# romanoshiliarhopoulos/Backgammon-Engine

Measured on AMD Instinct MI355X. Metric: self-play env steps/sec @65k concurrent games, higher is better.
Workload: dtype f32; 1 GPU; config3: 65 536 concurrent games per MI355X, greedy 198->128->1 value net (tdgammonNEW100k weights), auto-reset, Philox dice; games_per_gpu=65536, burnin_steps=160, parallelism=shard1, games_finished=2250605

## Files before the change

backgammon-engine_amd/csrc/bg_eval.h:

```cpp
#pragma once
#include "bg_board.h"
#include "bg_td_plan.h"
#include "bg_step_plan.h"

namespace bg {

constexpr int N_IN = 198, N_HID = 128;
constexpr int N_PARAMS = N_HID * N_IN + N_HID + N_HID + 1;
constexpr int K_STEPS = N_IN / 2;
constexpr int EVAL_LDS_BYTES = K_STEPS * 64 * 16;

typedef float floatx16 __attribute__((ext_vector_type(16)));

__device__ __forceinline__ float fast_sigmoid(float x)
{
    return __builtin_amdgcn_rcpf(1.0f + __builtin_amdgcn_exp2f(-1.44269504088896340736f * x));
}

__device__ __forceinline__ void best_atomic_max(unsigned long long *__restrict__ best, uint32_t game, float v, uint32_t key_turn,
                                                bool valid, int width)
{
    const int lane = threadIdx.x & 63;
    uint32_t bits = __float_as_uint(v);
    bits = (key_turn >> 31) ? ~bits : bits;
// ... 14 lines not shown
    uint32_t od[2][4];
    float tail[3];
};

__device__ __forceinline__ void decode_setup(const uint32_t (&p)[8], int h, RowDecode &r)
{
#pragma unroll
    for (int q = 0; q < 2; ++q) {
        const uint32_t b0 = p[4 * q] & PTS, b1 = p[4 * q + 1] & PTS, b2 = p[4 * q + 2] & PTS, b3 = p[4 * q + 3] & PTS;
        const uint32_t ge1 = b0 | b1 | b2 | b3;
        const uint32_t ge2 = b1 | b2 | b3;
        const uint32_t ge3 = (b0 & b1) | b2 | b3;
        const uint32_t ge4 = b2 | b3;
        const uint32_t s0 = ~b0, c0 = b0;
        const uint32_t s1 = b1 ^ c0, c1 = b1 & c0;
        const uint32_t s2 = ~(b2 ^ c1), c2 = b2 | c1;
        const uint32_t s3 = ~(b3 ^ c2);
        r.ev[q] = h ? ge2 : ge1;
        r.od[q][0] = h ? (s0 & ge4) : 0u;
        r.od[q][1] = h ? (s1 & ge4) : ge3;
        r.od[q][2] = h ? (s2 & ge4) : 0u;
        r.od[q][3] = h ? (s3 & ge4) : 0u;
    }
    const Side a{{p[0], p[1], p[2], p[3]}}, b{{p[4], p[5], p[6], p[7]}};
    const int turn = (p[0] & TURN_BIT) ? 1 : 0;
    r.tail[0] = (h == turn) ? 1.0f : 0.0f;
    r.tail[1] = 0.5f * (float)(h ? count_at(b, 25) : count_at(a, 0));
    r.tail[2] = (float)(h ? count_at(b, 0) : count_at(a, 25)) / 15.0f;
}

__device__ __forceinline__ float decode_even(const RowDecode &r, int q, int i)
{
    return (float)((r.ev[q] >> (i + 1)) & 1u);
}
__device__ __forceinline__ float decode_odd(const RowDecode &r, int q, int i)
{
    const int sh = i + 1;
    const uint32_t code = ((r.od[q][0] >> sh) & 1u) | (((r.od[q][1] >> sh) & 1u) << 1) |
                          (((r.od[q][2] >> sh) & 1u) << 2) | (((r.od[q][3] >> sh) & 1u) << 3);
    return 0.5f * (float)code;
}

inline void relayout_w1_f32(const float *w1 , float *wl )
{
    for (int s = 0; s < K_STEPS; ++s)
        for (int l = 0; l < 64; ++l)
            for (int c = 0; c < 4; ++c)
                wl[(s * 64 + l) * 4 + c] = w1[(32 * c + (l & 31)) * N_IN + 2 * s + (l >> 5)];
}

constexpr int EVAL_RED_STRIDE = 33;
constexpr int EVAL_RED_FLOATS = 32 * EVAL_RED_STRIDE;
constexpr int EVAL_LDS_TOTAL = EVAL_LDS_BYTES + (EVAL_THREADS / 64) * EVAL_RED_FLOATS * 4;

template <bool HIDDEN>
__global__ __launch_bounds__(EVAL_THREADS) void eval_rows_f32_kernel(
    const uint4 *__restrict__ rows, const unsigned long long *__restrict__ n_rows_ptr, long long n_rows_imm,
    unsigned long long *__restrict__ rows_eval_counter, const float4 *__restrict__ wl, const float *__restrict__ b1, const float *__restrict__ w2,
    const float *__restrict__ b2p, float *__restrict__ values, const uint2 *__restrict__ info,
    unsigned long long *__restrict__ best, unsigned long long *__restrict__ ksteps_counter)
{
    extern __shared__ float4 sW[];
    float *sRed = reinterpret_cast<float *>(sW + K_STEPS * 64) + (threadIdx.x >> 6) * EVAL_RED_FLOATS;
    for (int i = threadIdx.x; i < K_STEPS * 64; i += EVAL_THREADS) sW[i] = wl[i];
    __syncthreads();

    long long n_rows = n_rows_imm;
    if (n_rows_ptr) { const long long c = (long long)*n_rows_ptr; n_rows = c < n_rows_imm ? c : n_rows_imm; }
    if (rows_eval_counter && blockIdx.x == 0 && threadIdx.x == 0) atomicAdd(rows_eval_counter, (unsigned long long)n_rows);
    const long long n_tiles = (n_rows + 31) >> 5;
    const int lane = threadIdx.x & 63;
    const int r = lane & 31, h = lane >> 5;
    const long long wave = (long long)blockIdx.x * (EVAL_THREADS / 64) + (threadIdx.x >> 6);
    const long long n_waves = (long long)gridDim.x * (EVAL_THREADS / 64);

    constexpr float NL2E = -1.44269504088896340736f;
    float b1s[4], w2v[4];
#pragma unroll
    for (int c = 0; c < 4; ++c) { b1s[c] = NL2E * b1[32 * c + r]; w2v[c] = w2[32 * c + r]; }
    const float b2 = *b2p;

    uint32_t ksteps = 0;
    uint4 nx0 = make_uint4(0, 0, 0, 0), nx1 = make_uint4(0, 0, 0, 0);
    if (wave < n_tiles && wave * 32 + r < n_rows) { nx0 = rows[2 * (wave * 32 + r)]; nx1 = rows[2 * (wave * 32 + r) + 1]; }

    for (long long tile = wave; tile < n_tiles; tile += n_waves) {
        const uint32_t p[8] = {nx0.x, nx0.y, nx0.z, nx0.w, nx1.x, nx1.y, nx1.z, nx1.w};
        {
            const long long nrow = (tile + n_waves) * 32 + r;
            nx0 = make_uint4(0, 0, 0, 0); nx1 = make_uint4(0, 0, 0, 0);
            if (nrow < n_rows) { nx0 = rows[2 * nrow]; nx1 = rows[2 * nrow + 1]; }
        }
        RowDecode rd;
        decode_setup(p, h, rd);

        uint32_t live[4];
        {
            const uint32_t b0a = p[0] & PTS, b1a = p[1] & PTS, b2a = p[2] & PTS, b3a = p[3] & PTS;
            const uint32_t b0b = p[4] & PTS, b1b = p[5] & PTS, b2b = p[6] & PTS, b3b = p[7] & PTS;
            live[0] = b0a | b1a | b2a | b3a;
            live[1] = (b0a & b1a) | b2a | b3a;
            live[2] = b0b | b1b | b2b | b3b;
            live[3] = (b0b & b1b) | b2b | b3b;
#pragma unroll
            for (int m = 1; m < 64; m <<= 1) {
#pragma unroll
                for (int q = 0; q < 4; ++q) live[q] |= __shfl_xor(live[q], m, 64);
            }
#pragma unroll
            for (int q = 0; q < 4; ++q) live[q] = __builtin_amdgcn_readfirstlane(live[q]) >> 1;
            ksteps += (uint32_t)(__popc(live[0]) + __popc(live[1]) + __popc(live[2]) + __popc(live[3]) + 3);
        }

        floatx16 acc0 = {0}, acc1 = {0}, acc2 = {0}, acc3 = {0};
#define BG_MFMA4(aval, WV)                                                          \
    {                                                                                \
        acc0 = __builtin_amdgcn_mfma_f32_32x32x2f32((aval), (WV).x, acc0, 0, 0, 0);    \
        acc1 = __builtin_amdgcn_mfma_f32_32x32x2f32((aval), (WV).y, acc1, 0, 0, 0);    \
        acc2 = __builtin_amdgcn_mfma_f32_32x32x2f32((aval), (WV).z, acc2, 0, 0, 0);    \
        acc3 = __builtin_amdgcn_mfma_f32_32x32x2f32((aval), (WV).w, acc3, 0, 0, 0);    \
    }
        __builtin_amdgcn_s_setprio(2);
        const float4 *wp = sW + lane;
        float4 wa = wp[0 * 64], wb = wp[1 * 64], wc = wp[2 * 64], wd = wp[3 * 64];
#pragma unroll 2
        for (int i = 0; i < 24; ++i) {
            const int nb = (4 * i + 4) * 64;
            const float4 na = wp[nb], nbb = wp[nb + 64], nc = wp[nb + 128], nd = wp[i < 23 ? nb + 192 : nb + 128];
            const float a0 = decode_even(rd, 0, i);
            const float a2 = decode_even(rd, 1, i);
            if ((live[0] >> i) & 1u) BG_MFMA4(a0, wa);
            if ((live[1] >> i) & 1u) { const float a1 = decode_odd(rd, 0, i); BG_MFMA4(a1, wb); }
            if ((live[2] >> i) & 1u) BG_MFMA4(a2, wc);
            if ((live[3] >> i) & 1u) { const float a3 = decode_odd(rd, 1, i); BG_MFMA4(a3, wd); }
            wa = na; wb = nbb; wc = nc; wd = nd;
        }
        BG_MFMA4(rd.tail[0], wa);
        BG_MFMA4(rd.tail[1], wb);
        BG_MFMA4(rd.tail[2], wc);
#undef BG_MFMA4

        __builtin_amdgcn_s_setprio(0);
        if (HIDDEN) {
            float bb[4];
#pragma unroll
            for (int c = 0; c < 4; ++c) bb[c] = b1[32 * c + r];
#pragma unroll
            for (int j = 0; j < 16; ++j) {
                const long long orow = tile * 32 + (j & 3) + 8 * (j >> 2) + 4 * h;
                if (orow < n_rows) {
                    float *o = values + orow * N_HID + r;
                    o[0] = NL2E * (acc0[j] + bb[0]); o[32] = NL2E * (acc1[j] + bb[1]);
                    o[64] = NL2E * (acc2[j] + bb[2]); o[96] = NL2E * (acc3[j] + bb[3]);
                }
            }
            continue;
        }
        float part[16];
#pragma unroll
        for (int j = 0; j < 16; ++j) {
            const float s0 = __builtin_amdgcn_rcpf(1.0f + __builtin_amdgcn_exp2f(__builtin_fmaf(acc0[j], NL2E, b1s[0])));
            const float s1 = __builtin_amdgcn_rcpf(1.0f + __builtin_amdgcn_exp2f(__builtin_fmaf(acc1[j], NL2E, b1s[1])));
            const float s2 = __builtin_amdgcn_rcpf(1.0f + __builtin_amdgcn_exp2f(__builtin_fmaf(acc2[j], NL2E, b1s[2])));
            const float s3 = __builtin_amdgcn_rcpf(1.0f + __builtin_amdgcn_exp2f(__builtin_fmaf(acc3[j], NL2E, b1s[3])));
            part[j] = w2v[0] * s0 + w2v[1] * s1 + w2v[2] * s2 + w2v[3] * s3;
        }
#pragma unroll
        for (int q = 0; q < 4; ++q)
#pragma unroll
            for (int j = 0; j < 4; ++j) sRed[r * EVAL_RED_STRIDE + 8 * q + 4 * h + j] = part[4 * q + j];
        __builtin_amdgcn_wave_barrier();
        float sum = 0.0f;
#pragma unroll
        for (int c = 0; c < 16; ++c) sum += sRed[(16 * h + c) * EVAL_RED_STRIDE + r];
        sum += __shfl_xor(sum, 32, 64);
        __builtin_amdgcn_wave_barrier();
        {
            const long long orow = tile * 32 + r;
            const bool vrow = h == 0 && orow < n_rows;
            const float v = fast_sigmoid(sum + b2);
            if (vrow) values[orow] = v;
            if (info) {
                const uint2 inf = vrow ? info[orow] : make_uint2(0u, 0u);
                best_atomic_max(best, inf.x, v, inf.y, vrow, 32);
            }
        }
    }
    __shared__ unsigned int s_ksteps;
    if (threadIdx.x == 0) s_ksteps = 0;
    __syncthreads();
    if (lane == 0 && ksteps) atomicAdd(&s_ksteps, ksteps);
    __syncthreads();
    if (ksteps_counter && threadIdx.x == 0 && s_ksteps) atomicAdd(ksteps_counter, (unsigned long long)s_ksteps);
}

#ifndef BG_DW_STRIDE
#define BG_DW_STRIDE 132
#endif
constexpr int DW_STRIDE = BG_DW_STRIDE;
#if defined(BG_ROW_LAYOUT) && BG_ROW_LAYOUT == 1
constexpr int DW_ROWS = 198;
__host__ __device__ constexpr int delta_row(int f) { return f < 192 ? (f >> 3) + 24 * (f & 7) : f; }
__host__ __device__ constexpr int delta_row_board(int point, int k8) { return point + 24 * k8; }
#else
constexpr int DW_ROWS = 9 * 24 + 6;
__host__ __device__ constexpr int delta_row(int f) { return f < 192 ? 9 * (f >> 3) + (f & 7) : 216 + (f - 192); }
__host__ __device__ constexpr int delta_row_board(int point, int k8) { return 9 * point + k8; }
#endif
constexpr int DELTA_W_FLOATS = DW_ROWS * DW_STRIDE;
constexpr int DELTA_MAX = 16;
#ifndef BG_CTR_STRIDE
#define BG_CTR_STRIDE 16
#endif
constexpr int DELTA_LDS_TOTAL = (DELTA_W_FLOATS + N_HID) * 4 + (DELTA_THREADS / 64) * DELTA_MAX * 64 * 2;

inline void relayout_w1_delta(const float *w1 , float *wt )
{
    const float NL2E = -1.44269504088896340736f;
    for (int i = 0; i < DELTA_W_FLOATS; ++i) wt[i] = 0.0f;
    for (int f = 0; f < N_IN; ++f)
        for (int n = 0; n < N_HID; ++n) {
            float w = NL2E * w1[n * N_IN + f];
            if (f >= 196) w = w / 15.0f;
            wt[delta_row(f) * DW_STRIDE + n] = 0.5f * w;
        }
}

typedef float f32x2_t __attribute__((ext_vector_type(2)));
typedef float f32x4_t __attribute__((ext_vector_type(4)));
#define BG_DA_FMA(ACC, W) "v_pk_fma_f32 " ACC ", %16, " W ", " ACC " op_sel_hi:[0,1,1]\n\t"
#define BG_DA_BODY(O0, O1, O2, O3, O4, O5, O6, O7)                                                          \
        "ds_read_b128 v[108:111], %17 offset:" #O0 "\n\t"                                                  \
        "ds_read_b128 v[112:115], %17 offset:" #O1 "\n\t"                                                  \
        "ds_read_b128 v[116:119], %17 offset:" #O2 "\n\t"                                                  \
        "ds_read_b128 v[120:123], %17 offset:" #O3 "\n\t"                                                  \
        "ds_read_b128 v[124:127], %17 offset:" #O4 "\n\t"                                                  \
        "s_waitcnt lgkmcnt(4)\n\t" BG_DA_FMA("%0", "v[108:109]") BG_DA_FMA("%1", "v[110:111]")              \
        "ds_read_b128 v[108:111], %17 offset:" #O5 "\n\t"                                                  \
        "s_waitcnt lgkmcnt(4)\n\t" BG_DA_FMA("%2", "v[112:113]") BG_DA_FMA("%3", "v[114:115]")              \
        "ds_read_b128 v[112:115], %17 offset:" #O6 "\n\t"                                                  \
        "s_waitcnt lgkmcnt(4)\n\t" BG_DA_FMA("%4", "v[116:117]") BG_DA_FMA("%5", "v[118:119]")              \
        "ds_read_b128 v[116:119], %17 offset:" #O7 "\n\t"                                                  \
        "s_waitcnt lgkmcnt(4)\n\t" BG_DA_FMA("%6", "v[120:121]") BG_DA_FMA("%7", "v[122:123]")              \
        "s_waitcnt lgkmcnt(3)\n\t" BG_DA_FMA("%8", "v[124:125]") BG_DA_FMA("%9", "v[126:127]")              \
        "s_waitcnt lgkmcnt(2)\n\t" BG_DA_FMA("%10", "v[108:109]") BG_DA_FMA("%11", "v[110:111]")            \
        "s_waitcnt lgkmcnt(1)\n\t" BG_DA_FMA("%12", "v[112:113]") BG_DA_FMA("%13", "v[114:115]")            \
        "s_waitcnt lgkmcnt(0)\n\t" BG_DA_FMA("%14", "v[116:117]") "v_pk_fma_f32 %15, %16, v[118:119], %15 op_sel_hi:[0,1,1]"
template <int OFF>
__device__ __forceinline__ void delta_apply_32(f32x2_t (&a)[16], f32x2_t d2, uint32_t lds_addr)
{
    static_assert(OFF == 0 || OFF == 128, "two halves of a 64-unit pass");
#define BG_DA_OPS                                                                                                  \
        : "+v"(a[0]), "+v"(a[1]), "+v"(a[2]), "+v"(a[3]), "+v"(a[4]), "+v"(a[5]), "+v"(a[6]), "+v"(a[7]), "+v"(a[8]),  \
          "+v"(a[9]), "+v"(a[10]), "+v"(a[11]), "+v"(a[12]), "+v"(a[13]), "+v"(a[14]), "+v"(a[15])                 \
        : "v"(d2), "v"(lds_addr)                                                                                   \
        : "v108", "v109", "v110", "v111", "v112", "v113", "v114", "v115", "v116", "v117", "v118", "v119", "v120", "v121", \
          "v122", "v123", "v124", "v125", "v126", "v127", "memory"
    if (OFF == 0) asm volatile(BG_DA_BODY(0, 16, 32, 48, 64, 80, 96, 112) BG_DA_OPS);
    else asm volatile(BG_DA_BODY(128, 144, 160, 176, 192, 208, 224, 240) BG_DA_OPS);
#undef BG_DA_OPS
}
#undef BG_DA_BODY
#undef BG_DA_FMA

__device__ __forceinline__ void delta_entry(uint32_t ent, uint32_t base, f32x2_t &d2, uint32_t &addr)
{
    float d;
    asm("v_cvt_f32_i32_sdwa %0, sext(%2) dst_sel:DWORD dst_unused:UNUSED_PAD src0_sel:BYTE_1\n\t"
        "v_mul_u32_u24_sdwa %1, %3, %2 dst_sel:DWORD dst_unused:UNUSED_PAD src0_sel:DWORD src1_sel:BYTE_0\n\t"
        "v_add_u32_e32 %1, %4, %1"
        : "=&v"(d), "=&v"(addr)
        : "v"(ent), "s"((uint32_t)(DW_STRIDE * 4)), "s"(base));
    d2.x = d;
}

__device__ __forceinline__ f32x2_t delta_sigmoid_pair(f32x2_t a, f32x2_t w, f32x2_t sum)
{
    f32x2_t e = {__builtin_amdgcn_exp2f(a.x), __builtin_amdgcn_exp2f(a.y)};
    e = e + (f32x2_t){1.0f, 1.0f};
    const f32x2_t r = {__builtin_amdgcn_rcpf(e.x), __builtin_amdgcn_rcpf(e.y)};
    return __builtin_elementwise_fma(w, r, sum);
}

#if BG_DELTA_THREADS == 1024
#define BG_DELTA_BOUNDS __launch_bounds__(DELTA_THREADS)
#else
#define BG_DELTA_BOUNDS __launch_bounds__(DELTA_THREADS, 4)
#endif
__global__ BG_DELTA_BOUNDS void eval_rows_delta_kernel(
    const uint4 *__restrict__ rows, const unsigned long long *__restrict__ n_rows_ptr, long long n_rows_imm,
    unsigned long long *__restrict__ rows_eval_counter, const float4 *__restrict__ wt, const float *__restrict__ w2,
    const float *__restrict__ b2p, const uint4 *__restrict__ root_rows, const float *__restrict__ root_hidden,
    float *__restrict__ values, const uint2 *__restrict__ info, unsigned long long *__restrict__ best,
    unsigned long long *__restrict__ delta_counter, unsigned long long *__restrict__ zero_words, int n_zero_words,
    unsigned long long *__restrict__ err_word, unsigned long long err_bit, const unsigned long long *__restrict__ n_rows_b_ptr, long long b_base)
{
    if (zero_words && blockIdx.x == 0 && (int)threadIdx.x < n_zero_words) zero_words[threadIdx.x] = 0ull;
#ifdef BG_EVAL_WGCLOCK
    const unsigned long long wg_t0 = wall_clock64();
#endif
    extern __shared__ float4 sW[];
    float *sW2 = reinterpret_cast<float *>(sW) + DELTA_W_FLOATS;
    uint16_t *sList = reinterpret_cast<uint16_t *>(sW2 + N_HID) + (threadIdx.x >> 6) * (DELTA_MAX * 64);
    for (int i = threadIdx.x; i < DELTA_W_FLOATS / 4; i += DELTA_THREADS) sW[i] = wt[i];
    if (threadIdx.x < N_HID) sW2[threadIdx.x] = w2[threadIdx.x];
    __shared__ unsigned int s_ticket;
    if (threadIdx.x == 0) s_ticket = 0;
    __syncthreads();

    long long n_rows = n_rows_imm, na1 = 0, na2 = 0, na3 = 0;
    if (n_rows_ptr) {
        const long long lim = n_rows_b_ptr ? b_base : n_rows_imm;
        const long long c = (long long)*n_rows_ptr;
        n_rows = c < lim ? c : lim;
    }
    if (n_rows_b_ptr) {
        const long long c1 = (long long)n_rows_b_ptr[0], c2 = (long long)n_rows_b_ptr[BG_CTR_STRIDE], c3 = (long long)n_rows_b_ptr[2 * BG_CTR_STRIDE];
        na1 = c1 < b_base ? c1 : b_base; na2 = c2 < b_base ? c2 : b_base; na3 = c3 < b_base ? c3 : b_base;
    }
    if (rows_eval_counter && blockIdx.x == 0 && threadIdx.x == 0) atomicAdd(rows_eval_counter, (unsigned long long)(n_rows + na1 + na2 + na3));
#ifndef BG_ARENA_ORDER
#define BG_ARENA_ORDER 123
#endif
    constexpr int AO0 = (BG_ARENA_ORDER / 1000) % 10, AO1 = (BG_ARENA_ORDER / 100) % 10, AO2 = (BG_ARENA_ORDER / 10) % 10, AO3 = BG_ARENA_ORDER % 10;
    static_assert(((1 << AO0) | (1 << AO1) | (1 << AO2) | (1 << AO3)) == 15, "a permutation of 0123");
    const long long cnt_of[4] = {n_rows, na1, na2, na3};
    const long long c0 = cnt_of[AO0], c1 = cnt_of[AO1], c2 = cnt_of[AO2], c3 = cnt_of[AO3];
    const long long t1 = (c0 + 63) >> 6, t2 = t1 + ((c1 + 63) >> 6), t3 = t2 + ((c2 + 63) >> 6);
    const long long n_tiles = t3 + ((c3 + 63) >> 6);
    auto tile_rows = [&](long long t, long long &end) -> long long {
        if (t < t1) { end = AO0 * b_base + c0; return AO0 * b_base + t * 64; }
        if (t < t2) { end = AO1 * b_base + c1; return AO1 * b_base + (t - t1) * 64; }
        if (t < t3) { end = AO2 * b_base + c2; return AO2 * b_base + (t - t2) * 64; }
        end = AO3 * b_base + c3;
        return AO3 * b_base + (t - t3) * 64;
    };
    const int lane = threadIdx.x & 63;
    int rl, inv;
    {
        const int hl = lane & 31;
        const int g = (hl < 4 || (hl >= 12 && hl < 16) || (hl >= 20 && hl < 28)) ? 0 : 1;
        const int k = hl < 4 ? hl : hl < 12 ? hl - 4 : hl < 16 ? hl - 8 : hl < 20 ? hl - 8 : hl < 28 ? hl - 12 : hl - 16;
        rl = (lane & 32) + 16 * g + k;
        const int R = lane, gg = (R >> 4) & 1, kk = R & 15;
        inv = (R & 32) + (gg == 0 ? (kk < 4 ? kk : kk < 8 ? 8 + kk : 12 + kk) : (kk < 8 ? 4 + kk : kk < 12 ? 8 + kk : 16 + kk));
    }
    const long long t_hi = n_tiles;
    auto grab = [&]() -> long long {
        unsigned int t = 0;
        if (lane == 0) t = atomicAdd(&s_ticket, 1u);
        return (long long)blockIdx.x + (long long)__builtin_amdgcn_readfirstlane(t) * (long long)gridDim.x;
    };
    const float b2 = *b2p;
    constexpr float NL2E = -1.44269504088896340736f;
    uint32_t n_delta = 0;
    bool list_overflow = false;

    uint4 nx0 = make_uint4(0, 0, 0, 0), nx1 = make_uint4(0, 0, 0, 0);
    uint2 nxi = make_uint2(0u, 0u);
    long long tile = grab();
    long long row_end = 0, row_cur = tile_rows(tile, row_end) + rl;
    if (tile < t_hi && row_cur < row_end) { nx0 = rows[2 * row_cur]; nx1 = rows[2 * row_cur + 1]; nxi = info[row_cur]; }
    uint4 nr0 = root_rows[2 * (long long)nxi.x], nr1 = root_rows[2 * (long long)nxi.x + 1];
    while (tile < t_hi) {
        const long long next_tile = grab();
        const long long row = row_cur;
        const bool valid = row < row_end;
        const uint2 inf = nxi;
        const uint4 r0 = nr0, r1 = nr1;
        const f32x4_t *ah = reinterpret_cast<const f32x4_t *>(root_hidden + (long long)inf.x * N_HID);
        const uint32_t p[8] = {nx0.x & ~TURN_BIT, nx0.y, nx0.z, nx0.w, nx1.x, nx1.y, nx1.z, nx1.w};
        const uint32_t mover = (nx0.x & TURN_BIT) ? 1u : 0u;
        const uint32_t q[8] = {valid ? r0.x & ~TURN_BIT : 0u, valid ? r0.y : 0u, valid ? r0.z : 0u, valid ? r0.w : 0u,
                               valid ? r1.x : 0u, valid ? r1.y : 0u, valid ? r1.z : 0u, valid ? r1.w : 0u};
        {
            const long long nrow = tile_rows(next_tile, row_end) + rl;
            row_cur = nrow;
            nx0 = make_uint4(0, 0, 0, 0); nx1 = make_uint4(0, 0, 0, 0); nxi = make_uint2(0u, 0u);
            if (next_tile < t_hi && nrow < row_end) { nx0 = rows[2 * nrow]; nx1 = rows[2 * nrow + 1]; nxi = info[nrow]; }
        }

        uint32_t cnt = 0;
        uint16_t *lst = sList + lane;
#pragma unroll
        for (int e = 0; e < DELTA_MAX; ++e) lst[e * 64] = 0;
#if defined(BG_ABL) && (BG_ABL & 1)
        if (p[0] == 0xFFFFFFFFu)
#endif
        {
#define BG_PUSH(F, TYPE, M)                                                                          \
    {                                                                                                \
        if (cnt < DELTA_MAX) lst[cnt * 64] = (uint16_t)((uint32_t)(F) | ((uint32_t)(((TYPE) == 1 ? 1 : 2) * (M)) & 255u) << 8); \
        ++cnt;                                                                                       \
    }
#if !defined(BG_DECODE_MOVER_FIRST) || BG_DECODE_MOVER_FIRST
#pragma unroll
        for (int pass = 0; pass < 2; ++pass) {
            const uint32_t sd = mover ^ (uint32_t)pass;
            const uint32_t b0 = sd ? p[4] : p[0], b1 = sd ? p[5] : p[1], b2 = sd ? p[6] : p[2], b3 = sd ? p[7] : p[3];
            const uint32_t c0 = sd ? q[4] : q[0], c1 = sd ? q[5] : q[1], c2 = sd ? q[6] : q[2], c3 = sd ? q[7] : q[3];
            const uint32_t diff = (b0 ^ c0) | (b1 ^ c1) | (b2 ^ c2) | (b3 ^ c3);
            if (pass == 1 && __ballot(diff != 0u) == 0ull) break;
            const uint32_t ge_new[3] = {b0 | b1 | b2 | b3, b1 | b2 | b3, (b0 & b1) | b2 | b3};
            const uint32_t ge_old[3] = {c0 | c1 | c2 | c3, c1 | c2 | c3, (c0 & c1) | c2 | c3};
            const uint32_t side4 = 4u * sd;
#pragma unroll
            for (int k = 0; k < 3; ++k) {
                uint32_t x = (ge_new[k] ^ ge_old[k]) & PTS;
                while (x) {
                    const int pos = __ffs(x) - 1; x &= x - 1;
                    BG_PUSH(delta_row_board(pos - 1, 0) + side4 + (uint32_t)k, 0, ((ge_new[k] >> pos) & 1u) ? 1 : -1);
                }
            }
            uint32_t x4 = diff & PTS & ((b2 | b3) | (c2 | c3));
            const Side sn{{b0, b1, b2, b3}}, so{{c0, c1, c2, c3}};
            while (x4) {
                const int pos = __ffs(x4) - 1; x4 &= x4 - 1;
                const int n1 = count_at(sn, pos), n0 = count_at(so, pos);
                const int d = (n1 > 3 ? n1 - 3 : 0) - (n0 > 3 ? n0 - 3 : 0);
                if (d) BG_PUSH(delta_row_board(pos - 1, 0) + side4 + 3u, 1, d);
            }
            if (diff & 1u) {
                const int d = count_at(sn, 0) - count_at(so, 0);
                BG_PUSH(sd ? (uint32_t)delta_row(197) : (uint32_t)delta_row(194), 1, sd ? 2 * d : d);
            }
            if (diff & (1u << 25)) {
                const int d = count_at(sn, 25) - count_at(so, 25);
                BG_PUSH(sd ? (uint32_t)delta_row(195) : (uint32_t)delta_row(196), 1, sd ? d : 2 * d);
            }
        }
#else
#pragma unroll
        for (int sd = 0; sd < 2; ++sd) {
            const uint32_t b0 = p[4 * sd], b1 = p[4 * sd + 1], b2 = p[4 * sd + 2], b3 = p[4 * sd + 3];
            const uint32_t c0 = q[4 * sd], c1 = q[4 * sd + 1], c2 = q[4 * sd + 2], c3 = q[4 * sd + 3];
            const uint32_t diff = (b0 ^ c0) | (b1 ^ c1) | (b2 ^ c2) | (b3 ^ c3);
            const uint32_t ge_new[3] = {b0 | b1 | b2 | b3, b1 | b2 | b3, (b0 & b1) | b2 | b3};
            const uint32_t ge_old[3] = {c0 | c1 | c2 | c3, c1 | c2 | c3, (c0 & c1) | c2 | c3};
#pragma unroll
            for (int k = 0; k < 3; ++k) {
                uint32_t x = (ge_new[k] ^ ge_old[k]) & PTS;
                while (x) {
                    const int pos = __ffs(x) - 1; x &= x - 1;
                    BG_PUSH(delta_row_board(pos - 1, 4 * sd + k), 0, ((ge_new[k] >> pos) & 1u) ? 1 : -1);
                }
            }
            uint32_t x4 = diff & PTS & ((b2 | b3) | (c2 | c3));
            const Side sn{{b0, b1, b2, b3}}, so{{c0, c1, c2, c3}};
            while (x4) {
                const int pos = __ffs(x4) - 1; x4 &= x4 - 1;
                const int n1 = count_at(sn, pos), n0 = count_at(so, pos);
                const int d = (n1 > 3 ? n1 - 3 : 0) - (n0 > 3 ? n0 - 3 : 0);
                if (d) BG_PUSH(delta_row_board(pos - 1, 4 * sd + 3), 1, d);
            }
            if (diff & 1u) {
                const int d = count_at(sn, 0) - count_at(so, 0);
                BG_PUSH(delta_row(sd == 0 ? 194 : 197), sd == 0 ? 1 : 2, d);
            }
            if (diff & (1u << 25)) {
                const int d = count_at(sn, 25) - count_at(so, 25);
                BG_PUSH(delta_row(sd == 0 ? 196 : 195), sd == 0 ? 2 : 1, d);
            }
        }
#endif
        }
#undef BG_PUSH
        if (cnt > DELTA_MAX) { cnt = DELTA_MAX; list_overflow = true; }
        n_delta += cnt;
        uint32_t maxcnt = 0;
#pragma unroll
        for (int b = 4; b >= 0; --b) {
            const uint32_t t = maxcnt | (1u << b);
            if (__ballot(cnt >= t) != 0ull) maxcnt = t;
        }
#if defined(BG_ABL) && (BG_ABL & 2)
        maxcnt = maxcnt > 100 ? 1 : 0;
#endif
        __builtin_amdgcn_wave_barrier();

        f32x2_t sum2 = {0.0f, 0.0f};
        const f32x4_t *w2v = reinterpret_cast<const f32x4_t *>(sW2);
        const uint32_t sW_lds = (uint32_t)(uintptr_t)(__attribute__((address_space(3))) float4 *)sW;
#pragma unroll 1
        for (int c = 0; c < 2; ++c) {
            f32x2_t a[16], a2[16];
#if defined(BG_ABL) && (BG_ABL & 8)
#pragma unroll
            for (int j = 0; j < 16; ++j) { a[j] = (f32x2_t){0.25f * (float)j, 0.5f}; a2[j] = (f32x2_t){0.125f, -0.25f * (float)j}; }
            (void)ah;
#else
#pragma unroll
            for (int j = 0; j < 8; ++j) { const f32x4_t t = ah[16 * c + j]; a[2 * j] = t.lo; a[2 * j + 1] = t.hi; }
#pragma unroll
            for (int j = 0; j < 8; ++j) { const f32x4_t t = ah[16 * c + 8 + j]; a2[2 * j] = t.lo; a2[2 * j + 1] = t.hi; }
#endif
            if (c == 1) { nr0 = root_rows[2 * (long long)nxi.x]; nr1 = root_rows[2 * (long long)nxi.x + 1]; }
            uint32_t ent = lst[0];
            for (uint32_t e = 0; e < maxcnt; ++e) {
                const uint32_t nent = lst[(e + 1 < DELTA_MAX ? e + 1 : e) * 64];
                f32x2_t d2;
                uint32_t addr;
                delta_entry(ent, sW_lds + 256u * (uint32_t)c, d2, addr);
                delta_apply_32<0>(a, d2, addr);
                delta_apply_32<128>(a2, d2, addr);
                ent = nent;
            }
#if defined(BG_ABL) && (BG_ABL & 4)
#define BG_SIGP(A, W, S) __builtin_elementwise_fma(W, A, S)
#else
#define BG_SIGP(A, W, S) delta_sigmoid_pair(A, W, S)
#endif
#pragma unroll
            for (int j = 0; j < 8; ++j) {
                const f32x4_t w = w2v[16 * c + j];
                sum2 = BG_SIGP(a[2 * j], w.lo, sum2);
                sum2 = BG_SIGP(a[2 * j + 1], w.hi, sum2);
            }
#pragma unroll
            for (int j = 0; j < 8; ++j) {
                const f32x4_t w = w2v[16 * c + 8 + j];
                sum2 = BG_SIGP(a2[2 * j], w.lo, sum2);
                sum2 = BG_SIGP(a2[2 * j + 1], w.hi, sum2);
            }
#undef BG_SIGP
        }
        const float sum = sum2.x + sum2.y;
        __builtin_amdgcn_wave_barrier();
        {
            const float v = fast_sigmoid(sum + b2);
            if (valid) values[row] = v;
            best_atomic_max(best, __shfl(inf.x, inv, 64), __shfl(v, inv, 64), __shfl(inf.y, inv, 64), __shfl((int)valid, inv, 64) != 0, 64);
        }
        tile = next_tile;
    }
    __shared__ unsigned int s_nd;
    if (threadIdx.x == 0) s_nd = 0;
    __syncthreads();
    {
        uint32_t t = n_delta;
#pragma unroll
        for (int m = 1; m < 64; m <<= 1) t += __shfl_xor(t, m, 64);
        if (lane == 0 && t) atomicAdd(&s_nd, t);
    }
    __syncthreads();
    if (delta_counter && threadIdx.x == 0 && s_nd) atomicAdd(delta_counter, (unsigned long long)s_nd);
    if (err_word && __ballot(list_overflow) != 0ull && lane == 0) atomicOr(err_word, err_bit);
#ifdef BG_EVAL_WGCLOCK
    if (n_rows_ptr && threadIdx.x == 0) {
        values[n_rows_imm - 1 - (long long)blockIdx.x] = (float)(wall_clock64() - wg_t0) * 0.01f;
        values[n_rows_imm - 1 - (long long)gridDim.x - (long long)blockIdx.x] = (float)s_ticket;
        values[n_rows_imm - 1 - 10240 - (long long)blockIdx.x] = __uint_as_float((uint32_t)wg_t0);
        values[n_rows_imm - 1 - 11264 - (long long)blockIdx.x] = __uint_as_float((uint32_t)wall_clock64());
    }
#endif
}

constexpr int K16_STEPS = 13;
constexpr int EVAL16_W_BYTES = K16_STEPS * 4 * 64 * 16;
constexpr int EVAL16_LUT_BYTES = 16 * 8;
constexpr int EVAL16_LDS_TOTAL = EVAL16_W_BYTES + EVAL16_LUT_BYTES + (EVAL_THREADS / 64) * EVAL_RED_FLOATS * 4;
typedef __bf16 bf16x8 __attribute__((ext_vector_type(8)));

__host__ __device__ inline uint16_t f32_to_bf16_rne(float f)
{
    union { float f; uint32_t u; } c{f};
    return (uint16_t)((c.u + 0x7FFFu + ((c.u >> 16) & 1u)) >> 16);
}

inline void relayout_w1_bf16(const float *w1, uint16_t *wl)
{
    for (int s = 0; s < K16_STEPS; ++s)
        for (int c = 0; c < 4; ++c)
            for (int l = 0; l < 64; ++l)
                for (int j = 0; j < 8; ++j) {
                    const int f = 16 * s + 8 * (l >> 5) + j;
                    wl[((s * 4 + c) * 64 + l) * 8 + j] = f < N_IN ? f32_to_bf16_rne(w1[(32 * c + (l & 31)) * N_IN + f]) : 0;
                }
}
inline void make_count_lut(uint32_t *lut )
{
    for (int n = 0; n < 16; ++n) {
        const uint16_t e0 = n >= 1 ? 0x3F80 : 0, e1 = n >= 2 ? 0x3F80 : 0, e2 = n >= 3 ? 0x3F80 : 0;
        const uint16_t e3 = n >= 4 ? f32_to_bf16_rne(0.5f * (float)(n - 3)) : 0;
        lut[2 * n] = (uint32_t)e0 | ((uint32_t)e1 << 16);
        lut[2 * n + 1] = (uint32_t)e2 | ((uint32_t)e3 << 16);
    }
}

__global__ __launch_bounds__(EVAL_THREADS) void eval_rows_bf16_kernel(
    const uint4 *__restrict__ rows, const unsigned long long *__restrict__ n_rows_ptr, long long n_rows_imm,
    unsigned long long *__restrict__ rows_eval_counter, const uint4 *__restrict__ wl16, const uint2 *__restrict__ lut,
    const float *__restrict__ b1, const float *__restrict__ w2, const float *__restrict__ b2p, float *__restrict__ values,
    const uint2 *__restrict__ info, unsigned long long *__restrict__ best)
{
    extern __shared__ uint4 sW16[];
    uint2 *sLut = reinterpret_cast<uint2 *>(sW16 + K16_STEPS * 4 * 64);
    float *sRed = reinterpret_cast<float *>(sLut + 16) + (threadIdx.x >> 6) * EVAL_RED_FLOATS;
    for (int i = threadIdx.x; i < K16_STEPS * 4 * 64; i += EVAL_THREADS) sW16[i] = wl16[i];
    if (threadIdx.x < 16) sLut[threadIdx.x] = lut[threadIdx.x];
    __syncthreads();

    long long n_rows = n_rows_imm;
    if (n_rows_ptr) { const long long c = (long long)*n_rows_ptr; n_rows = c < n_rows_imm ? c : n_rows_imm; }
    if (rows_eval_counter && blockIdx.x == 0 && threadIdx.x == 0) atomicAdd(rows_eval_counter, (unsigned long long)n_rows);
    const long long n_tiles = (n_rows + 31) >> 5;
    const int lane = threadIdx.x & 63;
    const int r = lane & 31, h = lane >> 5;
    const long long wave = (long long)blockIdx.x * (EVAL_THREADS / 64) + (threadIdx.x >> 6);
    const long long n_waves = (long long)gridDim.x * (EVAL_THREADS / 64);
    constexpr float NL2E = -1.44269504088896340736f;
    float b1s[4], w2v[4];
#pragma unroll
    for (int c = 0; c < 4; ++c) { b1s[c] = NL2E * b1[32 * c + r]; w2v[c] = w2[32 * c + r]; }
    const float b2 = *b2p;

    uint4 nx0 = make_uint4(0, 0, 0, 0), nx1 = make_uint4(0, 0, 0, 0);
    if (wave < n_tiles && wave * 32 + r < n_rows) { nx0 = rows[2 * (wave * 32 + r)]; nx1 = rows[2 * (wave * 32 + r) + 1]; }

    for (long long tile = wave; tile < n_tiles; tile += n_waves) {
        const uint32_t p[8] = {nx0.x, nx0.y, nx0.z, nx0.w, nx1.x, nx1.y, nx1.z, nx1.w};
        {
            const long long nrow = (tile + n_waves) * 32 + r;
            nx0 = make_uint4(0, 0, 0, 0); nx1 = make_uint4(0, 0, 0, 0);
            if (nrow < n_rows) { nx0 = rows[2 * nrow]; nx1 = rows[2 * nrow + 1]; }
        }
        const Side sa{{p[0], p[1], p[2], p[3]}}, sb{{p[4], p[5], p[6], p[7]}};
        floatx16 acc0 = {0}, acc1 = {0}, acc2 = {0}, acc3 = {0};
        const uint4 *wp = sW16 + lane;
#pragma unroll 4
        for (int s = 0; s < 12; ++s) {
            const int pos = 2 * s + h + 1;
            const uint2 l0 = sLut[count_at(sa, pos)], l1 = sLut[count_at(sb, pos)];
            union { uint4 u; bf16x8 v; } a, w0, w1, w2r, w3;
            a.u = make_uint4(l0.x, l0.y, l1.x, l1.y);
            w0.u = wp[(s * 4 + 0) * 64]; w1.u = wp[(s * 4 + 1) * 64]; w2r.u = wp[(s * 4 + 2) * 64]; w3.u = wp[(s * 4 + 3) * 64];
            acc0 = __builtin_amdgcn_mfma_f32_32x32x16_bf16(a.v, w0.v, acc0, 0, 0, 0);
            acc1 = __builtin_amdgcn_mfma_f32_32x32x16_bf16(a.v, w1.v, acc1, 0, 0, 0);
            acc2 = __builtin_amdgcn_mfma_f32_32x32x16_bf16(a.v, w2r.v, acc2, 0, 0, 0);
            acc3 = __builtin_amdgcn_mfma_f32_32x32x16_bf16(a.v, w3.v, acc3, 0, 0, 0);
        }
        {
            const int turn = (p[0] & TURN_BIT) ? 1 : 0;
            const uint32_t t0 = turn == 0 ? 0x3F80u : 0u, t1 = turn == 0 ? 0u : 0x3F80u;
            const uint32_t bar1 = f32_to_bf16_rne(0.5f * (float)count_at(sa, 0)), bar2 = f32_to_bf16_rne(0.5f * (float)count_at(sb, 25));
            const uint32_t off1 = f32_to_bf16_rne((float)count_at(sa, 25) / 15.0f), off2 = f32_to_bf16_rne((float)count_at(sb, 0) / 15.0f);
            union { uint4 u; bf16x8 v; } a, w0, w1, w2r, w3;
            a.u = h ? make_uint4(0, 0, 0, 0) : make_uint4(t0 | (t1 << 16), bar1 | (bar2 << 16), off1 | (off2 << 16), 0u);
            w0.u = wp[(12 * 4 + 0) * 64]; w1.u = wp[(12 * 4 + 1) * 64]; w2r.u = wp[(12 * 4 + 2) * 64]; w3.u = wp[(12 * 4 + 3) * 64];
            acc0 = __builtin_amdgcn_mfma_f32_32x32x16_bf16(a.v, w0.v, acc0, 0, 0, 0);
            acc1 = __builtin_amdgcn_mfma_f32_32x32x16_bf16(a.v, w1.v, acc1, 0, 0, 0);
            acc2 = __builtin_amdgcn_mfma_f32_32x32x16_bf16(a.v, w2r.v, acc2, 0, 0, 0);
            acc3 = __builtin_amdgcn_mfma_f32_32x32x16_bf16(a.v, w3.v, acc3, 0, 0, 0);
        }
        float part[16];
#pragma unroll
        for (int j = 0; j < 16; ++j) {
            const float s0 = __builtin_amdgcn_rcpf(1.0f + __builtin_amdgcn_exp2f(__builtin_fmaf(acc0[j], NL2E, b1s[0])));
            const float s1 = __builtin_amdgcn_rcpf(1.0f + __builtin_amdgcn_exp2f(__builtin_fmaf(acc1[j], NL2E, b1s[1])));
            const float s2 = __builtin_amdgcn_rcpf(1.0f + __builtin_amdgcn_exp2f(__builtin_fmaf(acc2[j], NL2E, b1s[2])));
            const float s3 = __builtin_amdgcn_rcpf(1.0f + __builtin_amdgcn_exp2f(__builtin_fmaf(acc3[j], NL2E, b1s[3])));
            part[j] = w2v[0] * s0 + w2v[1] * s1 + w2v[2] * s2 + w2v[3] * s3;
        }
#pragma unroll
        for (int q = 0; q < 4; ++q)
#pragma unroll
            for (int j = 0; j < 4; ++j) sRed[r * EVAL_RED_STRIDE + 8 * q + 4 * h + j] = part[4 * q + j];
        __builtin_amdgcn_wave_barrier();
        float sum = 0.0f;
#pragma unroll
        for (int c = 0; c < 16; ++c) sum += sRed[(16 * h + c) * EVAL_RED_STRIDE + r];
        sum += __shfl_xor(sum, 32, 64);
        __builtin_amdgcn_wave_barrier();
        {
            const long long orow = tile * 32 + r;
            const bool vrow = h == 0 && orow < n_rows;
            const float v = fast_sigmoid(sum + b2);
            if (vrow) values[orow] = v;
            if (info) {
                const uint2 inf = vrow ? info[orow] : make_uint2(0u, 0u);
                best_atomic_max(best, inf.x, v, inf.y, vrow, 32);
            }
        }
    }
}

#ifndef BG_ROOT3_PHASE_STEPS
#define BG_ROOT3_PHASE_STEPS 7
#endif
constexpr int ROOT3_PHASE_STEPS = BG_ROOT3_PHASE_STEPS;
constexpr int ROOT3_PHASES = (K16_STEPS + ROOT3_PHASE_STEPS - 1) / ROOT3_PHASE_STEPS;
constexpr int ROOT3_PART_U4 = K16_STEPS * 4 * 64;
constexpr int ROOT3_LDS_TOTAL = 3 * ROOT3_PHASE_STEPS * 4 * 64 * 16 + EVAL16_LUT_BYTES;

inline void relayout_w1_bf16x3(const float *w1, uint16_t *wl)
{
    static const int tail_map[8] = {192, 193, 194, 195, 196, 197, -1, -1};
    for (int s = 0; s < K16_STEPS; ++s)
        for (int c = 0; c < 4; ++c)
            for (int l = 0; l < 64; ++l)
                for (int j = 0; j < 8; ++j) {
                    int f = 16 * s + 8 * (l >> 5) + j;
                    if (s == 12) f = (l >> 5) == 0 ? tail_map[j] : -1;
                    float w = f >= 0 && f < N_IN ? w1[(32 * c + (l & 31)) * N_IN + f] : 0.0f;
                    if (f >= 196) w = w / 15.0f;
                    const size_t o = (((size_t)s * 4 + c) * 64 + l) * 8 + j;
                    for (int part = 0; part < 3; ++part) {
                        const uint16_t b = f32_to_bf16_rne(w);
                        union { uint32_t u; float f; } cv;
                        cv.u = (uint32_t)b << 16;
                        w -= cv.f;
                        wl[(size_t)part * ROOT3_PART_U4 * 8 + o] = b;
                    }
                }
}

struct RootRowsFetch {
    const uint4 *rows;
    __device__ __forceinline__ bool get(long long R, uint4 &u0, uint4 &u1) const { u0 = rows[2 * R]; u1 = rows[2 * R + 1]; return true; }
};
struct TrajRowsFetch {
    const uint4 *rows; const int4 *gmeta; long long t, n_lanes, T;
    __device__ __forceinline__ bool get(long long R, uint4 &u0, uint4 &u1) const
    {
        const int4 gm = gmeta[R >> 1];
        const long long tt = t - gm.w + (R & 1);
        if (tt >= gm.y || tt >= T) return false;
        long long lr = tt + (gm.z >> 1);
        if (lr >= T) lr -= T;
        const uint4 *src = rows + (lr * n_lanes + gm.x) * 2;
        u0 = src[0]; u1 = src[1];
        return true;
    }
};

template <class Fetch, bool LOG2E_SCALE>
__device__ __forceinline__ void root3_body(const Fetch fetch, long long n_rows, const uint4 *__restrict__ wl3, const uint2 *__restrict__ lut,
                                           const float *__restrict__ b1, float *__restrict__ hidden)
{
    extern __shared__ uint4 sW3[];
    uint2 *sLut = reinterpret_cast<uint2 *>(sW3 + 3 * ROOT3_PHASE_STEPS * 4 * 64);
    if (threadIdx.x < 16) sLut[threadIdx.x] = lut[threadIdx.x];
    const long long n_tiles = (n_rows + 31) >> 5;
    const int lane = threadIdx.x & 63;
    const int r = lane & 31, h = lane >> 5;
    const long long wave = (long long)blockIdx.x * (ROOT3_THREADS / 64) + (threadIdx.x >> 6);
    const long long n_waves = (long long)gridDim.x * (ROOT3_THREADS / 64);
    constexpr float NL2E = -1.44269504088896340736f;
    constexpr int PH = ROOT3_PHASE_STEPS * 4 * 64;

    for (long long base = 0; base < n_tiles; base += n_waves) {
        const long long tile = base + wave;
        const bool has = tile < n_tiles;
        uint32_t p[8] = {0, 0, 0, 0, 0, 0, 0, 0};
        bool row_ok = false;
        if (has && tile * 32 + r < n_rows) {
            uint4 u0, u1;
            if (fetch.get(tile * 32 + r, u0, u1)) {
                row_ok = true;
                p[0] = u0.x; p[1] = u0.y; p[2] = u0.z; p[3] = u0.w; p[4] = u1.x; p[5] = u1.y; p[6] = u1.z; p[7] = u1.w;
            }
        }
        const Side sa{{p[0], p[1], p[2], p[3]}}, sb{{p[4], p[5], p[6], p[7]}};
        floatx16 acc0 = {0}, acc1 = {0}, acc2 = {0}, acc3 = {0};
#pragma unroll 1
        for (int phase = 0; phase < ROOT3_PHASES; ++phase) {
            const int s0 = phase * ROOT3_PHASE_STEPS;
            const int ns = K16_STEPS - s0 < ROOT3_PHASE_STEPS ? K16_STEPS - s0 : ROOT3_PHASE_STEPS;
            __syncthreads();
            for (int i = threadIdx.x; i < 3 * ns * 4 * 64; i += ROOT3_THREADS) {
                const int part = i / (ns * 4 * 64), o = i - part * (ns * 4 * 64);
                sW3[part * PH + o] = wl3[(size_t)part * ROOT3_PART_U4 + (size_t)s0 * 4 * 64 + o];
            }
            __syncthreads();
            if (has) {
                const uint4 *wp = sW3 + lane;
                for (int k = 0; k < ns; ++k) {
                    const int s = s0 + k;
                    union { uint4 u; bf16x8 v; } a;
                    if (s < 12) {
                        const int pos = 2 * s + h + 1;
                        const uint2 l0 = sLut[count_at(sa, pos)], l1 = sLut[count_at(sb, pos)];
                        a.u = make_uint4(l0.x, l0.y, l1.x, l1.y);
                    } else {
                        const int turn = (p[0] & TURN_BIT) ? 1 : 0;
                        const uint32_t t0 = (turn == 0 && row_ok) ? 0x3F80u : 0u, t1 = (turn == 0 || !row_ok) ? 0u : 0x3F80u;
                        const uint32_t bar1 = f32_to_bf16_rne(0.5f * (float)count_at(sa, 0)), bar2 = f32_to_bf16_rne(0.5f * (float)count_at(sb, 25));
                        const uint32_t off1 = f32_to_bf16_rne((float)count_at(sa, 25)), off2 = f32_to_bf16_rne((float)count_at(sb, 0));
                        a.u = h ? make_uint4(0, 0, 0, 0) : make_uint4(t0 | (t1 << 16), bar1 | (bar2 << 16), off1 | (off2 << 16), 0u);
                    }
#pragma unroll
                    for (int part = 0; part < 3; ++part) {
                        union { uint4 u; bf16x8 v; } w0, w1, w2r, w3;
                        const uint4 *q = wp + part * PH + k * 4 * 64;
                        w0.u = q[0]; w1.u = q[64]; w2r.u = q[128]; w3.u = q[192];
                        acc0 = __builtin_amdgcn_mfma_f32_32x32x16_bf16(a.v, w0.v, acc0, 0, 0, 0);
                        acc1 = __builtin_amdgcn_mfma_f32_32x32x16_bf16(a.v, w1.v, acc1, 0, 0, 0);
                        acc2 = __builtin_amdgcn_mfma_f32_32x32x16_bf16(a.v, w2r.v, acc2, 0, 0, 0);
                        acc3 = __builtin_amdgcn_mfma_f32_32x32x16_bf16(a.v, w3.v, acc3, 0, 0, 0);
                    }
                }
            }
        }
        if (has) {
            float bb[4];
#pragma unroll
            for (int c = 0; c < 4; ++c) bb[c] = b1[32 * c + r];
#pragma unroll
            for (int j = 0; j < 16; ++j) {
                const long long orow = tile * 32 + (j & 3) + 8 * (j >> 2) + 4 * h;
                if (orow < n_rows) {
                    float *o = hidden + orow * N_HID + r;
                    constexpr float SC = LOG2E_SCALE ? NL2E : 1.0f;
                    o[0] = SC * (acc0[j] + bb[0]); o[32] = SC * (acc1[j] + bb[1]);
                    o[64] = SC * (acc2[j] + bb[2]); o[96] = SC * (acc3[j] + bb[3]);
                }
            }
        }
    }
}

#ifdef BGAMD_EXPERIMENTAL
__global__ __launch_bounds__(ROOT3_THREADS) void root_hidden_bf16x3_kernel(
    const uint4 *__restrict__ rows, long long n_rows, const uint4 *__restrict__ wl3, const uint2 *__restrict__ lut,
    const float *__restrict__ b1, float *__restrict__ hidden)
{
    root3_body<RootRowsFetch, true>(RootRowsFetch{rows}, n_rows, wl3, lut, b1, hidden);
}
#endif

__global__ __launch_bounds__(ROOT3_THREADS) void traj_hidden_bf16x3_kernel(
    const uint4 *__restrict__ rows, const int4 *__restrict__ gmeta, long long t, long long n_lanes, long long T, long long n_rows,
    const uint4 *__restrict__ wl3, const uint2 *__restrict__ lut, const float *__restrict__ b1, float *__restrict__ hidden)
{
    root3_body<TrajRowsFetch, false>(TrajRowsFetch{rows, gmeta, t, n_lanes, T}, n_rows, wl3, lut, b1, hidden);
}

constexpr int ROOT3D_THREADS = 256;
#ifdef BGAMD_EXPERIMENTAL
__global__ __launch_bounds__(ROOT3D_THREADS) void traj_hidden_direct_kernel(
    const uint4 *__restrict__ rows, const int4 *__restrict__ gmeta, long long t, long long n_lanes, long long T, long long n_rows,
    const uint4 *__restrict__ wl3, const uint2 *__restrict__ lut, const float *__restrict__ b1, float *__restrict__ hidden)
{
    __shared__ uint2 sLut[16];
    if (threadIdx.x < 16) sLut[threadIdx.x] = lut[threadIdx.x];
    const int lane = threadIdx.x & 63, c = threadIdx.x >> 6;
    const int r = lane & 31, h = lane >> 5;
    const long long tile = blockIdx.x;
    const TrajRowsFetch fetch{rows, gmeta, t, n_lanes, T};
    uint32_t p[8] = {0, 0, 0, 0, 0, 0, 0, 0};
    bool row_ok = false;
    if (tile * 32 + r < n_rows) {
        uint4 u0, u1;
        if (fetch.get(tile * 32 + r, u0, u1)) {
            row_ok = true;
            p[0] = u0.x; p[1] = u0.y; p[2] = u0.z; p[3] = u0.w; p[4] = u1.x; p[5] = u1.y; p[6] = u1.z; p[7] = u1.w;
// ... 236 lines not shown
```

Before: 528.2 million env steps/s.

## Overlap LDS weight staging with counter and first-tile row loads in delta eval

```diff
diff --git a/backgammon-engine_amd/csrc/bg_eval.h b/backgammon-engine_amd/csrc/bg_eval.h
--- a/backgammon-engine_amd/csrc/bg_eval.h
+++ b/backgammon-engine_amd/csrc/bg_eval.h
@@ -340,22 +340,36 @@
     extern __shared__ float4 sW[];
     float *sW2 = reinterpret_cast<float *>(sW) + DELTA_W_FLOATS;
     uint16_t *sList = reinterpret_cast<uint16_t *>(sW2 + N_HID) + (threadIdx.x >> 6) * (DELTA_MAX * 64);
-    for (int i = threadIdx.x; i < DELTA_W_FLOATS / 4; i += DELTA_THREADS) sW[i] = wt[i];
-    if (threadIdx.x < N_HID) sW2[threadIdx.x] = w2[threadIdx.x];
     __shared__ unsigned int s_ticket;
-    if (threadIdx.x == 0) s_ticket = 0;
-    __syncthreads();
+    constexpr int STAGE_STEPS = (DELTA_W_FLOATS / 4 + DELTA_THREADS - 1) / DELTA_THREADS;
+    auto stage = [&](int k0, int k1) {
+#pragma unroll
+        for (int k = k0; k < k1; ++k) {
+            const int i = k * DELTA_THREADS + (int)threadIdx.x;
+            if (i < DELTA_W_FLOATS / 4) sW[i] = wt[i];
+        }
+    };
+    unsigned long long cr0 = 0, cr1 = 0, cr2 = 0, cr3 = 0;
+    if (n_rows_ptr) cr0 = *n_rows_ptr;
+    if (n_rows_b_ptr) { cr1 = n_rows_b_ptr[0]; cr2 = n_rows_b_ptr[BG_CTR_STRIDE]; cr3 = n_rows_b_ptr[2 * BG_CTR_STRIDE]; }
+    const float b2 = *b2p;
+    const float w2_mine = threadIdx.x < N_HID ? w2[threadIdx.x] : 0.0f;
+    stage(0, STAGE_STEPS / 3);
 
     long long n_rows = n_rows_imm, na1 = 0, na2 = 0, na3 = 0;
     if (n_rows_ptr) {
         const long long lim = n_rows_b_ptr ? b_base : n_rows_imm;
-        const long long c = (long long)*n_rows_ptr;
+        const long long c = (long long)cr0;
         n_rows = c < lim ? c : lim;
     }
     if (n_rows_b_ptr) {
-        const long long c1 = (long long)n_rows_b_ptr[0], c2 = (long long)n_rows_b_ptr[BG_CTR_STRIDE], c3 = (long long)n_rows_b_ptr[2 * BG_CTR_STRIDE];
+        const long long c1 = (long long)cr1, c2 = (long long)cr2, c3 = (long long)cr3;
         na1 = c1 < b_base ? c1 : b_base; na2 = c2 < b_base ? c2 : b_base; na3 = c3 < b_base ? c3 : b_base;
     }
+#ifdef BG_EVAL_WGCLOCK
+    asm volatile("s_waitcnt lgkmcnt(0)" : "+s"(na3) : : "memory");
+    const unsigned long long wg_t_counters = wall_clock64();
+#endif
     if (rows_eval_counter && blockIdx.x == 0 && threadIdx.x == 0) atomicAdd(rows_eval_counter, (unsigned long long)(n_rows + na1 + na2 + na3));
 #ifndef BG_ARENA_ORDER
 #define BG_ARENA_ORDER 123
@@ -364,14 +378,14 @@
     static_assert(((1 << AO0) | (1 << AO1) | (1 << AO2) | (1 << AO3)) == 15, "a permutation of 0123");
     const long long cnt_of[4] = {n_rows, na1, na2, na3};
     const long long c0 = cnt_of[AO0], c1 = cnt_of[AO1], c2 = cnt_of[AO2], c3 = cnt_of[AO3];
-    const long long t1 = (c0 + 63) >> 6, t2 = t1 + ((c1 + 63) >> 6), t3 = t2 + ((c2 + 63) >> 6);
-    const long long n_tiles = t3 + ((c3 + 63) >> 6);
-    auto tile_rows = [&](long long t, long long &end) -> long long {
-        if (t < t1) { end = AO0 * b_base + c0; return AO0 * b_base + t * 64; }
-        if (t < t2) { end = AO1 * b_base + c1; return AO1 * b_base + (t - t1) * 64; }
-        if (t < t3) { end = AO2 * b_base + c2; return AO2 * b_base + (t - t2) * 64; }
+    const int t1 = (int)((c0 + 63) >> 6), t2 = t1 + (int)((c1 + 63) >> 6), t3 = t2 + (int)((c2 + 63) >> 6);
+    const int n_tiles = t3 + (int)((c3 + 63) >> 6);
+    auto tile_rows = [&](int t, long long &end) -> long long {
+        if (t < t1) { end = AO0 * b_base + c0; return AO0 * b_base + (long long)t * 64; }
+        if (t < t2) { end = AO1 * b_base + c1; return AO1 * b_base + (long long)(t - t1) * 64; }
+        if (t < t3) { end = AO2 * b_base + c2; return AO2 * b_base + (long long)(t - t2) * 64; }
         end = AO3 * b_base + c3;
-        return AO3 * b_base + (t - t3) * 64;
+        return AO3 * b_base + (long long)(t - t3) * 64;
     };
     const int lane = threadIdx.x & 63;
     int rl, inv;
@@ -383,25 +397,39 @@
         const int R = lane, gg = (R >> 4) & 1, kk = R & 15;
         inv = (R & 32) + (gg == 0 ? (kk < 4 ? kk : kk < 8 ? 8 + kk : 12 + kk) : (kk < 8 ? 4 + kk : kk < 12 ? 8 + kk : 16 + kk));
     }
-    const long long t_hi = n_tiles;
-    auto grab = [&]() -> long long {
+    const int t_hi = n_tiles;
+    auto grab = [&]() -> int {
         unsigned int t = 0;
         if (lane == 0) t = atomicAdd(&s_ticket, 1u);
-        return (long long)blockIdx.x + (long long)__builtin_amdgcn_readfirstlane(t) * (long long)gridDim.x;
+        return (int)blockIdx.x + (int)__builtin_amdgcn_readfirstlane(t) * (int)gridDim.x;
     };
-    const float b2 = *b2p;
     constexpr float NL2E = -1.44269504088896340736f;
     uint32_t n_delta = 0;
     bool list_overflow = false;
 
     uint4 nx0 = make_uint4(0, 0, 0, 0), nx1 = make_uint4(0, 0, 0, 0);
     uint2 nxi = make_uint2(0u, 0u);
-    long long tile = grab();
+    int tile = (int)blockIdx.x + (int)__builtin_amdgcn_readfirstlane(threadIdx.x >> 6) * (int)gridDim.x;
     long long row_end = 0, row_cur = tile_rows(tile, row_end) + rl;
-    if (tile < t_hi && row_cur < row_end) { nx0 = rows[2 * row_cur]; nx1 = rows[2 * row_cur + 1]; nxi = info[row_cur]; }
+    {
+        const bool ok = tile < t_hi && row_cur < row_end;
+        const long long r = ok ? row_cur : 0;
+        nx0 = rows[2 * r]; nx1 = rows[2 * r + 1]; nxi = info[r];
+        stage(STAGE_STEPS / 3, 2 * STAGE_STEPS / 3);
+        if (!ok) { nx0 = make_uint4(0, 0, 0, 0); nx1 = make_uint4(0, 0, 0, 0); nxi = make_uint2(0u, 0u); }
+    }
     uint4 nr0 = root_rows[2 * (long long)nxi.x], nr1 = root_rows[2 * (long long)nxi.x + 1];
+    stage(2 * STAGE_STEPS / 3, STAGE_STEPS);
+    if (threadIdx.x < N_HID) sW2[threadIdx.x] = w2_mine;
+    if (threadIdx.x == 0) s_ticket = DELTA_THREADS / 64;
+    __syncthreads();
+#ifdef BG_EVAL_WGCLOCK
+    const unsigned long long wg_t_staged = wall_clock64();
+    bool wg_first_pass = true;
+    unsigned long long wg_t_gather = 0;
+#endif
     while (tile < t_hi) {
-        const long long next_tile = grab();
+        const int next_tile = grab();
         const long long row = row_cur;
         const bool valid = row < row_end;
         const uint2 inf = nxi;
@@ -534,6 +562,13 @@
 #endif
             if (c == 1) { nr0 = root_rows[2 * (long long)nxi.x]; nr1 = root_rows[2 * (long long)nxi.x + 1]; }
             uint32_t ent = lst[0];
+#ifdef BG_EVAL_WGCLOCK
+            if (wg_first_pass) {
+                asm volatile("s_waitcnt vmcnt(0) lgkmcnt(0)" ::: "memory");
+                wg_t_gather = wall_clock64();
+                wg_first_pass = false;
+            }
+#endif
             for (uint32_t e = 0; e < maxcnt; ++e) {
                 const uint32_t nent = lst[(e + 1 < DELTA_MAX ? e + 1 : e) * 64];
                 f32x2_t d2;
@@ -589,6 +624,9 @@
         values[n_rows_imm - 1 - (long long)gridDim.x - (long long)blockIdx.x] = (float)s_ticket;
         values[n_rows_imm - 1 - 10240 - (long long)blockIdx.x] = __uint_as_float((uint32_t)wg_t0);
         values[n_rows_imm - 1 - 11264 - (long long)blockIdx.x] = __uint_as_float((uint32_t)wall_clock64());
+        values[n_rows_imm - 1 - 14336 - (long long)blockIdx.x] = (float)(wg_t_counters - wg_t0) * 0.01f;
+        values[n_rows_imm - 1 - 14336 - 256 - (long long)blockIdx.x] = (float)(wg_t_staged - wg_t0) * 0.01f;
+        values[n_rows_imm - 1 - 14336 - 512 - (long long)blockIdx.x] = wg_t_gather ? (float)(wg_t_gather - wg_t0) * 0.01f : 0.0f;
     }
 #endif
 }
```

After: 533.4 million env steps/s, median of 6. Within noise of the previous version (+1.0%).
